# henriChevreux/distillation_trajectories

Hardware: AMD Instinct MI355X
Metric: trajectory-timesteps/sec (B×T U-Net fwd) at 16×16 T=50 (higher is better)
Workload: dtype f32 (fp32-accurate; convolutions: exact 3-plane bf16 operand split on bf16 MFMA with fp32 accumulate, or native fp32 MFMA, chosen per layer)

## Files before the change

### distillation_trajectories_amd/csrc/build.py

```python
import os
import shutil
import subprocess
import sys

HERE = os.path.dirname(os.path.abspath(__file__))
SOURCES = ["dt_conv.hip", "dt_conv_bf16.hip", "dt_conv_strip.hip", "dt_layers.hip", "dt_update.hip", "dt_metrics.hip", "dt_fused.hip", "dt_profile.hip", "dt_unet.hip",
           "dt_unet_forward.hip", "dt_unet_tune.hip", "dt_sample.hip", "dt_featnet.hip", "dt_inception.hip", "dt_pca.hip", "dt_fid.hip", "dt_lpips.hip", "dt_tsne.hip", "dt_quality.hip", "dt_quality_stream.hip", "dt_edit.hip", "dt_rng.hip"]
HEADERS = ["dt_internal.h", "dt_conv_forms.h", "dt_conv_rows.h", "dt_batch.h", "dt_dense64.h", "dt_quality_math.h", "dt_featnet.h", "dt_conv_epilogue.h", "dt_conv_walk.h", "dt_update_math.h", "dt_fused.h", "dt_unet.h", "dt_unet_layout.h", os.path.join("..", "..", "include", "dt_hip.h"),
           os.path.join("..", "..", "include", "dt_hip_noise.h"),
           os.path.join("..", "..", "include", "dt_hip_inception.h"),
           os.path.join("..", "..", "include", "dt_hip_pca.h"),
           os.path.join("..", "..", "include", "dt_hip_fid.h"),
           os.path.join("..", "..", "include", "dt_hip_fid_cov.h"),
           os.path.join("..", "..", "include", "dt_hip_lpips.h"),
           os.path.join("..", "..", "include", "dt_hip_tsne.h"),
           os.path.join("..", "..", "include", "dt_hip_quality.h"),
           os.path.join("..", "..", "include", "dt_hip_quality_stream.h"),
           os.path.join("..", "..", "include", "dt_hip_edit.h"),
           os.path.join("..", "..", "include", "dt_hip_rng.h")]
LIB = os.path.join(HERE, "libdt_hip.so")
ARCH = "gfx950"


def hipcc_path():
    for cand in (os.environ.get("HIPCC"), "/opt/rocm/bin/hipcc", shutil.which("hipcc")):
        if cand and os.path.exists(cand):
            return cand
    raise RuntimeError("hipcc not found (looked at $HIPCC, /opt/rocm/bin/hipcc, PATH)")


OBJ_DIR = os.path.join(HERE, "_build")
FLAGS = [f"--offload-arch={ARCH}", "-O3", "-std=c++17", "-fPIC", "-Wall", "-Wno-unused-function"]


def _newer(target, deps):
    if not os.path.exists(target):
        return True
    t = os.path.getmtime(target)
    return any(os.path.getmtime(d) > t for d in deps)


def is_stale():
    deps = [os.path.join(HERE, f) for f in SOURCES + HEADERS] + [os.path.abspath(__file__)]
    return _newer(LIB, deps)


def build(force=False, verbose=False):
    if not force and not is_stale():
        return LIB
    from concurrent.futures import ThreadPoolExecutor
    os.makedirs(OBJ_DIR, exist_ok=True)
    hipcc = hipcc_path()
    common = [os.path.join(HERE, f) for f in HEADERS] + [os.path.abspath(__file__)]

    def compile_one(src):
        obj = os.path.join(OBJ_DIR, src.replace(".hip", ".o"))
        path = os.path.join(HERE, src)
        if not force and not _newer(obj, [path] + common):
            return obj, None
# ... 85 lines not shown
```

### distillation_trajectories_amd/csrc/dt_conv.hip

```cpp
#include "dt_conv_walk.h"

namespace dt {

template <int BM, int BN>
__global__ __launch_bounds__(256, 4) void conv_gemm_kernel(const ConvParams p) {
  constexpr ConvForm F = *find_conv_form(KIND_FP32, BM, BN);
  constexpr int WN = F.wn();
  constexpr int MI = F.mi(), NI = F.ni();
  constexpr int A_PER = BM / 64, B_PER = BN / 64;
  constexpr int STAGE = (BM + BN) * 16;
  constexpr int LDS_FLOATS = 2 * STAGE > F.stage_floats() ? 2 * STAGE : F.stage_floats();
  static_assert(F.wm() == 2 && WN == 2 && MI * 64 == BM && NI * 64 == BN && LDS_FLOATS >= F.stage_floats(), "wave layout, epilogue stage");
  __shared__ __attribute__((aligned(16))) float lds[LDS_FLOATS];

  const int tid = threadIdx.x, lane = tid & 63, wave = tid >> 6;
  const int wm = wave / WN, wn = wave % WN;
  const int half = lane >> 5, l31 = lane & 31;
  const int m0 = blockIdx.x * BM, n0 = blockIdx.y * BN;
  const int HW = p.H * p.W;
  const ConvRowMath rm = kernarg_row_math();

  int a_off[A_PER], a_off2[A_PER], a_y[A_PER], a_x[A_PER];
  bool a_ok[A_PER];
  int a_lds[A_PER];
// ... 50 lines not shown
      for (int j = 0; j < B_PER; ++j) rb[j] = *reinterpret_cast<const f32x4 *>(wt + j * 1024);
      k.next();
    }
    if (it >= 0) {
      if (k.at_midpoint(p, it)) conv_midpoint<MI, NI>(p, acc, n0, wn, l31);
      const float *A = lds + (it & 1) * STAGE, *B = A + BM * 16;
#pragma unroll
      for (int s = 0; s < 2; ++s) {
        f32x4 fa[MI], fb[NI];
#pragma unroll
        for (int mi = 0; mi < MI; ++mi)
          fa[mi] = *reinterpret_cast<const f32x4 *>(A + a_row[mi] * 16 + (((2 * s + half) ^ ((a_row[mi] >> 2) & 3)) << 2));
#pragma unroll
        for (int ni = 0; ni < NI; ++ni)
          fb[ni] = *reinterpret_cast<const f32x4 *>(B + b_row[ni] * 16 + (((2 * s + half) ^ ((b_row[ni] >> 2) & 3)) << 2));
#pragma unroll
        for (int i = 0; i < 4; ++i)
#pragma unroll
          for (int mi = 0; mi < MI; ++mi)
#pragma unroll
            for (int ni = 0; ni < NI; ++ni) {
              acc[mi][ni] = __builtin_amdgcn_mfma_f32_32x32x2f32(fa[mi][i], fb[ni][i], acc[mi][ni], 0, 0, 0);
            }
      }
    }
    if (more) {
      float *A = lds + ((it + 1) & 1) * STAGE, *B = A + BM * 16;
#pragma unroll
      for (int j = 0; j < A_PER; ++j) *reinterpret_cast<f32x4 *>(A + a_lds[j]) = ra[j];
#pragma unroll
      for (int j = 0; j < B_PER; ++j) *reinterpret_cast<f32x4 *>(B + (tid + j * 256) * 4) = rb[j];
    }
    __syncthreads();
  }

  conv_epilogue<BM, BN, 1, false, true>(p, acc, lds, m0, n0, wm, wn, half, l31);
}

int launch_splitk_epilogue(const ConvParams &p, hipStream_t s);

#define DT_GEMM_ROW(cls, kind, bm, bn, kc, wk) {{kind, bm, bn, kc, wk, cls}, conv_gemm_kernel<bm, bn>},
static const ConvKernel kGemmKernels[] = {DT_CONV_FORMS_FP32(DT_GEMM_ROW)};

int launch_conv(const ConvParams &p_in, hipStream_t s) {
  ConvParams p = p_in;
  if (!p.in || !p.w || !p.scale || !p.shift || !p.out) return DT_E_NULL;
  if (p.H < 1 || p.W < 1) return DT_E_SHAPE;
  p.rm = make_row_math(p.H, p.W, p.m_per_tb, p.x3_imgs);
  if (p.cin_p % 16 || p.cout_p % 16 || p.n_p % kNPad || p.M <= 0) return DT_E_SHAPE;
  if ((long long)p.M * p.cin_p >= (1ll << 31) || (long long)p.M * p.cout_p * (p.n_dup > 1 ? p.n_dup : 1) >= (1ll << 31)) return DT_E_SHAPE;
  if (const int st = conv_admissible(p)) return st;
  {
    const double flops = 2.0 * p.M * (double)p.cout_real * ((double)p.cin_real * p.ksize * p.ksize + (p.in2 ? p.cin2_real : 0));
    ProfileScope prof(find_conv_form(p.kind, p.bm, p.bn)->cls, flops, 4.0 * p.M * ((double)p.cin_real + p.cout_real), s);
    if (p.kind == KIND_FP32) {
      conv_kernel_of(kGemmKernels, p).fn<<<dim3((p.M + p.bm - 1) / p.bm, p.n_p / p.bn, p.splits), 256, 0, s>>>(p);
      DT_LAUNCH_CHECK();
    } else if (const int st = is_strip(p.kind) ? launch_conv_strip(p, s) : launch_conv_bf16x6(p, s)) return st;
  }
  return p.splits > 1 ? launch_splitk_epilogue(p, s) : DT_OK;
}


bool conv_choice_valid(const ConvChoice &c, int slot, int n_p) {
  if (!find_conv_form(c.kind, c.bm, c.bn) || n_p % c.bn) return false;
  if (c.splits < 1 || c.splits > 9 || c.splits == 5 || c.splits == 6 || c.splits == 7) return false;
  return !c.fuse || (slot == 2 && c.splits == 1);
}

static ConvChoice heuristic_choice(int M, int n_p, int taps) {
  ConvChoice c{};
  c.bn = n_p % 128 == 0 ? 128 : 64;
  const long long blocks128 = (long long)((M + 127) / 128) * (n_p / c.bn);
  c.bm = blocks128 >= 512 ? 128 : 64;
  const long long blocks = (long long)((M + c.bm - 1) / c.bm) * (n_p / c.bn);
  c.splits = 1;
  if (taps == 9 && M <= kSplitMaxRows && blocks < 384) c.splits = blocks * 3 >= 384 ? 3 : 9;
  c.fuse = c.splits == 1;
  return c;
}

ConvChoice resolve_conv_choice(const ConvLayer &L, const ConvChoice *req, int precision) {
  ConvChoice c = req ? *req : heuristic_choice(L.M, L.n_p, L.splittable ? L.taps : 1);
  const int cc = L.cin_p >> 4;
  if (!req) {
    c.kind = precision == DT_PREC_FP32 ? KIND_FP32 : KIND_BF16;
    if (c.kind == KIND_BF16 && L.taps == 9 && strip_reaches(L.W)) {
      c.kind = KIND_STRIP;
      c.splits = c.splits == 9 ? (cc % 8 == 0 ? 8 : (cc % 4 == 0 ? 4 : 1)) : (c.splits == 3 ? (cc % 4 == 0 ? 4 : (cc % 2 == 0 ? 2 : 1)) : 1);
    }
  }
  if (c.kind == 2) c.kind = KIND_BF16;
  if (is_strip(c.kind) && (L.taps != 9 || !strip_reaches(L.W))) c.kind = KIND_BF16;
  if (c.kind == KIND_STRIPK && !find_conv_form(c.kind, c.bm, c.bn)) c.kind = KIND_STRIP2;
  if (c.bm == 256 && !find_conv_form(c.kind, c.bm, c.bn)) c.bm = 128;
  if (!L.splittable) c.splits = 1;
  const ConvForm *f = find_conv_form(c.kind, c.bm, c.bn);
  if (is_strip(c.kind) ? !chunks_fit(cc, pack_chunks(L.cin_p), c.splits * (f ? f->kc : 1)) : (L.taps * cc) % c.splits != 0)
    c.splits = 1;
  c.fuse = L.foldable && c.fuse && c.splits == 1;
  return c;
}

int conv_admissible(const ConvParams &p) {
  const int cc = p.cin_p >> 4;
  const ConvForm *f = find_conv_form(p.kind, p.bm, p.bn);
  if (!f || p.n_p % p.bn) return DT_E_ARG;
  if (p.splits < 1 || (p.splits > 1 && !p.slab)) return DT_E_ARG;
  if (p.ccw < cc || (p.in2 && p.ccw2 < (p.cin2_p >> 4))) return DT_E_ARG;
  if (p.in2 && (p.splits != 1 || !p.w2 || !p.bias2 || p.cin2_p % 16)) return DT_E_ARG;
  if (!is_strip(p.kind)) return (p.tap_hi - p.tap_lo) * cc % p.splits ? DT_E_ARG : DT_OK;
  if (p.ksize != 3 || p.tap_lo != 0 || p.tap_hi != 9 || !chunks_fit(cc, p.ccw, p.splits * f->kc)) return DT_E_ARG;
  if (p.in2 && !chunks_fit(p.cin2_p >> 4, p.ccw2, f->kc)) return DT_E_ARG;
  return f->reaches(p.W) ? DT_OK : DT_E_SHAPE;
}

template <int S>
__device__ inline float4 splitk_finish(const ConvParams &p, unsigned m, int n, size_t slab_stride) {
  const size_t o = (size_t)m * p.cout_p + n;
  float4 a;
  if (S > 0) {
    float4 part[S > 0 ? S : 1];
#pragma unroll
    for (int z = 0; z < S; ++z) part[z] = *reinterpret_cast<const float4 *>(p.slab + z * slab_stride + o);
    a = part[0];
#pragma unroll
    for (int z = 1; z < S; ++z) { a.x += part[z].x; a.y += part[z].y; a.z += part[z].z; a.w += part[z].w; }
  } else {
    a = *reinterpret_cast<const float4 *>(p.slab + o);
    for (int z = 1; z < p.splits; ++z) {
      const float4 b = *reinterpret_cast<const float4 *>(p.slab + z * slab_stride + o);
      a.x += b.x; a.y += b.y; a.z += b.z; a.w += b.w;
    }
  }
  const float4 sc = *reinterpret_cast<const float4 *>(p.scale + n), sh = *reinterpret_cast<const float4 *>(p.shift + n);
  float4 v = make_float4(a.x * sc.x + sh.x, a.y * sc.y + sh.y, a.z * sc.z + sh.z, a.w * sc.w + sh.w);
  if (p.relu) { v.x = fmaxf(v.x, 0.f); v.y = fmaxf(v.y, 0.f); v.z = fmaxf(v.z, 0.f); v.w = fmaxf(v.w, 0.f); }
  if (p.tb) {
    const float4 t = *reinterpret_cast<const float4 *>(p.tb + (size_t)row_tb((int)m, p.rm) * p.tb_stride + n);
    v.x += t.x; v.y += t.y; v.z += t.z; v.w += t.w;
  }
  if (p.add) {
    const float4 t = *reinterpret_cast<const float4 *>(p.add + o);
    v.x += t.x; v.y += t.y; v.z += t.z; v.w += t.w;
  }
  *reinterpret_cast<float4 *>(p.out + o) = v;
  return v;
}

template <int S, bool POOL>
__global__ __launch_bounds__(256) void splitk_epilogue_kernel(const ConvParams p) {
  const unsigned c4 = (unsigned)p.cout_p >> 2;
  const size_t slab_stride = (size_t)p.M * p.cout_p;
  const bool pow2 = (c4 & (c4 - 1)) == 0;
  const int sh4 = 31 - __builtin_clz(c4);
  if (!POOL) {
    const unsigned total = (unsigned)p.M * c4;
    for (unsigned i = blockIdx.x * blockDim.x + threadIdx.x; i < total; i += gridDim.x * blockDim.x) {
// ... 114 lines not shown
```

### distillation_trajectories_amd/csrc/dt_conv_forms.h

```cpp
#pragma once
#include <stddef.h>

namespace dt {

enum ConvKind {
  KIND_FP32 = 0,
  KIND_BF16 = 1,
  KIND_STRIP = 3,
  KIND_STRIP2 = 4,
  KIND_STRIPK = 5,
};
constexpr bool is_strip(int kind) { return kind >= KIND_STRIP; }

constexpr int strip_halo(int W, int bm) { return bm % W == 0 ? W : W + 1; }

constexpr int conv_real_channel(int cp, int cin, int cin_p, int split_c, int split_cp) {
  return cp < split_cp ? (cp < split_c ? cp : -1) : (cp < cin_p && split_c + (cp - split_cp) < cin ? split_c + (cp - split_cp) : -1);
}

enum ConvClass {
  KC_CONV_128x128 = 0, KC_CONV_128x64, KC_CONV_64x128, KC_CONV_64x64,
  KC_CONVB_128x128, KC_CONVB_128x64, KC_CONVB_64x128, KC_CONVB_64x64,
  KC_CONVS_128x128, KC_CONVS_128x64, KC_CONVS_64x128, KC_CONVS_64x64, KC_CONVS_256x64, KC_CONVS_K128x64, KC_CONVS_K64x64, KC_CONVS_K64x128,
  KC_CONV_COUNT
};

#define DT_CONV_FORMS_FP32(X)                    \
  X(KC_CONV_128x128, KIND_FP32, 128, 128, 1, 1)  \
  X(KC_CONV_128x64, KIND_FP32, 128, 64, 1, 1)    \
  X(KC_CONV_64x128, KIND_FP32, 64, 128, 1, 1)    \
  X(KC_CONV_64x64, KIND_FP32, 64, 64, 1, 1)
#define DT_CONV_FORMS_BF16(X)                    \
  X(KC_CONVB_128x128, KIND_BF16, 128, 128, 1, 1) \
  X(KC_CONVB_128x64, KIND_BF16, 128, 64, 1, 1)   \
  X(KC_CONVB_64x128, KIND_BF16, 64, 128, 1, 1)   \
  X(KC_CONVB_64x64, KIND_BF16, 64, 64, 1, 1)
#define DT_CONV_FORMS_STRIPK(X)                   \
  X(KC_CONVS_K64x128, KIND_STRIPK, 64, 128, 2, 2) \
  X(KC_CONVS_K64x64, KIND_STRIPK, 64, 64, 4, 4)   \
  X(KC_CONVS_K128x64, KIND_STRIPK, 128, 64, 2, 2)
#define DT_CONV_FORMS_STRIP2(X)                    \
  X(KC_CONVS_256x64, KIND_STRIP2, 256, 64, 2, 1)   \
  X(KC_CONVS_128x128, KIND_STRIP2, 128, 128, 2, 1) \
  X(KC_CONVS_128x64, KIND_STRIP2, 128, 64, 2, 1)   \
  X(KC_CONVS_64x128, KIND_STRIP2, 64, 128, 2, 1)   \
  X(KC_CONVS_64x64, KIND_STRIP2, 64, 64, 2, 1)
#define DT_CONV_FORMS_STRIP(X)                    \
  X(KC_CONVS_256x64, KIND_STRIP, 256, 64, 1, 1)   \
  X(KC_CONVS_128x128, KIND_STRIP, 128, 128, 1, 1) \
  X(KC_CONVS_128x64, KIND_STRIP, 128, 64, 1, 1)   \
  X(KC_CONVS_64x128, KIND_STRIP, 64, 128, 1, 1)   \
  X(KC_CONVS_64x64, KIND_STRIP, 64, 64, 1, 1)
#define DT_CONV_FORMS_ALL_STRIP(X) DT_CONV_FORMS_STRIPK(X) DT_CONV_FORMS_STRIP2(X) DT_CONV_FORMS_STRIP(X)

struct ConvForm {
  int kind, bm, bn, kc, wk, cls;

  constexpr int wn() const { return wk > 1 ? bn / 64 : (bm == 256 ? 1 : 2); }
  constexpr int wm() const { return 4 / (wn() * wk); }
  constexpr int mi() const { return bm / (32 * wm()); }
  constexpr int ni() const { return bn / (32 * wn()); }
  constexpr int kw() const { return kc / wk; }

  constexpr int ap() const { return bm == 256 ? 3 : (kc == 4 ? 1 : 2); }
  constexpr int max_w() const { return kc == 4 ? 31 : 63; }
// ... 44 lines not shown
```

### distillation_trajectories_amd/csrc/dt_internal.h

```cpp
#pragma once
#include <hip/hip_runtime.h>
#include <stddef.h>
#include <stdint.h>

#include "../../include/dt_hip.h"
#include "dt_conv_forms.h"
#include "dt_conv_rows.h"
#include "dt_unet_layout.h"

#define DT_HIP_TRY(expr)                         \
  do {                                           \
    hipError_t _e = (expr);                      \
    if (_e != hipSuccess) return (int)_e;        \
  } while (0)
#define DT_LAUNCH_CHECK()                        \
  do {                                           \
    hipError_t _e = hipGetLastError();           \
    if (_e != hipSuccess) return (int)_e;        \
  } while (0)

namespace dt {

enum KernelClass {
  KC_SPLITK_EPILOGUE = KC_CONV_COUNT, KC_FIRST_CONV, KC_POOL, KC_UPCAT, KC_HEAD, KC_HEAD_UP, KC_TIME_BIAS, KC_UPDATE, KC_METRICS,
  KC_WASSERSTEIN, KC_RESAMPLE, KC_FUSED, KC_PAIR_METRICS,
  KC_COUNT
};
struct ProfileScope {
  ProfileScope(int cls, double flops, double bytes, hipStream_t s);
  ~ProfileScope();
  int slot;
  hipStream_t stream;
  void *end_event;
};
bool profiling_on();

__device__ inline void bilinear_src(int dst, int in, int out, int &i0, int &i1, float &l0, float &l1) {
#pragma clang fp contract(off)
  const float scale = out > 1 ? (float)(in - 1) / (float)(out - 1) : 0.f;
  const float src = scale * (float)dst;
  i0 = (int)src;
  i1 = i0 + (i0 < in - 1 ? 1 : 0);
  l1 = src - (float)i0;
  l0 = 1.f - l1;
}
__device__ inline float bilinear_blend(float v00, float v01, float v10, float v11, float wy0, float wy1, float wx0, float wx1) {
  const float top = fmaf(wx1, v01, wx0 * v00), bot = fmaf(wx1, v11, wx0 * v10);
  return fmaf(wy1, bot, wy0 * top);
}

inline int grid_blocks(size_t total, int cap) { return (int)((total + 255) / 256 < (size_t)cap ? (total + 255) / 256 : (size_t)cap); }
inline bool chunks_fit(int cc, int ccw, int div) { return div >= 1 && round_up(cc, div) <= ccw; }

struct ConvParams {
  const float *in;
  const float *w;
  const float *scale;
  const float *shift;
  const float *tb;
  const float *add;
  float *out;
  int M, H, W;
  int cin_p, cout_p, n_p;
  int cin_real, cout_real;
  int ksize;
  int tap_lo, tap_hi;
  int relu;
  int tb_stride;
  int m_per_tb;
  int splits;
  float *slab;
  int bm, bn;
  int kind;
  const float *x3;
  const float *w3;
  int x3_hw, x3_imgs, x3_c;
  const float *in2;
  const float *w2;
  const float *bias2;
  int cin2_p, cin2_real;
  float *pool_out;
  const float *in_b, *in2_b;
  int cc_a, b_stride;
  const float *head_w, *head_b;
  float *head_out;
  int head_c, head_cin;
  const float *tbc;
  int n_dup, dup_rows;
  int dup_skip;
  int skip_out;
  int dup_stage2;
  int ccw, ccw2;
  ConvRowMath rm;
};

int launch_conv(const ConvParams &p, hipStream_t s);
int launch_conv_bf16x6(const ConvParams &p, hipStream_t s);
int launch_conv_strip(const ConvParams &p, hipStream_t s);
struct ConvKernel { ConvForm form; void (*fn)(ConvParams); };
template <size_t N>
inline const ConvKernel &conv_kernel_of(const ConvKernel (&table)[N], const ConvParams &p) {
  for (const ConvKernel &k : table)
    if (k.form.kind == p.kind && k.form.bm == p.bm && k.form.bn == p.bn) return k;
  return table[0];
}
int launch_pack_conv_bf16x3(const float *w_oihw, void *wp, int cout, int cin, int ksize, int cin_p, int cin_w, int n_p,
                            int split_c, int split_cp, hipStream_t s);

struct ConvChoice { int bm, bn, splits, kind, fuse; };
struct ConvLayer {
  int M, W;
  int n_p, cin_p;
  int taps;
  bool splittable;
  bool foldable;
};
inline bool strip_reaches(int W) { return find_conv_form(KIND_STRIP, 64, 64)->reaches(W); }
bool conv_choice_valid(const ConvChoice &c, int slot, int n_p);
ConvChoice resolve_conv_choice(const ConvLayer &L, const ConvChoice *req, int precision);
int conv_admissible(const ConvParams &p);

int launch_pack_conv(const float *w_oihw, float *wp, int cout, int cin, int ksize, int cin_p, int n_p,
                     int split_c, int split_cp, hipStream_t s);
int launch_fold_bn(const float *conv_b, const float *g, const float *b, const float *mean, const float *var,
                   float *scale, float *shift, int cout, int n_p, hipStream_t s);
int launch_pack_linear_rows(const float *w, const float *b, float *wp, float *bp, int out, int in, int out_p,
                            hipStream_t s);

int launch_first_conv(const float *x, const float *wf, const float *scale, const float *shift, const float *tb, int tb_stride,
                      int tb_div, float *out, int B, int n_pass, int C, int H, int W, int cout, int cout_p, hipStream_t s);
int launch_pack_first_conv(const float *w_oihw, float *wf, int cout, int C, int cout_p, hipStream_t s);
int launch_pack_tap_major(const float *w_oihw, float *w2t, int cout, int cin, int cp, hipStream_t s);
int launch_maxpool(const float *in, float *out, int Bt, int H, int W, int cp, hipStream_t s);
int launch_upcat(const float *lo, const float *skip, float *out, int Bt, int h, int w, int c1p, int c2p,
                 hipStream_t s);
int launch_head(const float *lo, const float *w, const float *bias, float *lowres, int Bt, int h, int w_, int cp, int C, int c_real,
                hipStream_t s);
int launch_head_upsample(const float *lowres, float *eps, int Bt, int h, int w_, int C, hipStream_t s);
int launch_pack_res3(const float *w, const float *b, float *w3, int cout, int C, int n_p, hipStream_t s);
struct MaskArgs {
  const float *mask;
  const int32_t *mask_row;
  const float *known;
  const int32_t *known_row;
};
int launch_cfg_update_lowres(int rule, const float *x, const float *lowres_u, const float *lowres_c, const float *z,
                             const int32_t *z_row, long long z_shift, const float coef[4], int has_noise, const float *w,
                             float w_scalar, float *out, int B, int C, int H, int W, int b_single, hipStream_t s,
                             const MaskArgs &mk = MaskArgs{});

struct TembWeights {
  const float *freqs;
  const float *w1, *b1;
  const float *wc0, *bc0;
  const float *wc2, *bc2;
  const float *wt, *bt;
  int D, half, tb_stride;
  int tb_cols;
  const float *w2t;
  int c0p;
};
int launch_time_bias(const TembWeights &tw, const int32_t *t, const float *cond, const uint8_t *present, int rows,
                     float *out, hipStream_t s);

}
```

### distillation_trajectories_amd/csrc/dt_profile.hip

```cpp
#include <atomic>
#include <mutex>
#include <vector>

#include "dt_internal.h"

using namespace dt;

namespace {
struct ProfRecord { hipEvent_t a, b; int cls; double flops, bytes; };
struct Profiler {
  std::mutex mu;
  std::atomic<bool> on{false};
  std::vector<ProfRecord> rec;
  std::vector<hipEvent_t> pool;
  size_t used = 0;
  hipEvent_t get() {
    if (used == pool.size()) {
      hipEvent_t e;
      if (hipEventCreate(&e) != hipSuccess) return nullptr;
      pool.push_back(e);
    }
    return pool[used++];
  }
} g_prof;
const char *kClassName[KC_COUNT - KC_CONV_COUNT] = {
    "splitk_epilogue_kernel", "first_conv_kernel", "maxpool_kernel", "upcat_kernel", "head_kernel", "head_upsample_kernel",
    "time_bias_kernel", "cfg_update_kernel", "traj_metrics_kernel", "wasserstein_kernel", "resampled_distance_kernel",
    "unet_fused_kernel", "pair_metrics_kernel"};
const char *class_name(int cls) {
  switch (cls) {
#define DT_GEMM(c, kind, bm, bn, kc, wk) case c: return "conv_gemm_kernel<" #bm "," #bn ">";
#define DT_BF16(c, kind, bm, bn, kc, wk) case c: return "conv_gemm_bf16x6_kernel<" #bm "," #bn ">";
#define DT_STRIP(c, kind, bm, bn, kc, wk) case c: return "conv_strip_bf16x6_kernel<" #bm "," #bn ">";
#define DT_STRIPK(c, kind, bm, bn, kc, wk) case c: return "conv_strip_bf16x6_kernel<" #bm "," #bn ",K" #kc ">";
    DT_CONV_FORMS_FP32(DT_GEMM) DT_CONV_FORMS_BF16(DT_BF16) DT_CONV_FORMS_STRIP(DT_STRIP) DT_CONV_FORMS_STRIPK(DT_STRIPK)
    default: return kClassName[cls - KC_CONV_COUNT];
  }
}
}

namespace dt {
ProfileScope::ProfileScope(int cls, double flops, double bytes, hipStream_t s) : slot(-1), stream(s), end_event(nullptr) {
  if (!g_prof.on.load(std::memory_order_relaxed)) return;
  hipEvent_t a;
  {
    std::lock_guard<std::mutex> lock(g_prof.mu);
    if (!g_prof.on.load(std::memory_order_relaxed)) return;
    a = g_prof.get();
    hipEvent_t b = g_prof.get();
    if (!a || !b) return;
    g_prof.rec.push_back(ProfRecord{a, b, cls, flops, bytes});
    slot = (int)g_prof.rec.size() - 1;
    end_event = b;
  }
  (void)hipEventRecord(a, s);
}
ProfileScope::~ProfileScope() {
  if (slot < 0) return;
  (void)hipEventRecord((hipEvent_t)end_event, stream);
}
bool profiling_on() { return g_prof.on.load(); }
}

extern "C" {

__global__ void profile_marker_kernel(int) {}

int dt_profile_marker(int id, void *stream) {
  profile_marker_kernel<<<1, 64, 0, (hipStream_t)stream>>>(id);
  DT_LAUNCH_CHECK();
  return DT_OK;
}

int dt_profile_begin(void) {
  std::lock_guard<std::mutex> lock(g_prof.mu);
  g_prof.rec.clear();
  g_prof.used = 0;
  g_prof.on = true;
  return DT_OK;
}

// ... 25 lines not shown
```

### distillation_trajectories_amd/csrc/dt_unet.h

```cpp
#pragma once
#include <mutex>
#include <vector>

#include "dt_fused.h"

namespace dt {

struct ConvW {
  float *w, *wb;
  float *scale, *shift;
};
struct BlockW {
  ConvW c[3];
  float *w3;
};

struct TunedShape {
  FwdShape shape;
  ConvChoice c[kBlocks][3];
};

struct LoopGraph {
  std::vector<unsigned char> key;
  hipGraphExec_t exec = nullptr;
  hipGraph_t graph = nullptr;
  LoopGraph() = default;
  LoopGraph(LoopGraph &&o) noexcept : key(std::move(o.key)), exec(o.exec), graph(o.graph) { o.exec = nullptr; o.graph = nullptr; }
  LoopGraph &operator=(LoopGraph &&o) noexcept {
    std::swap(key, o.key); std::swap(exec, o.exec); std::swap(graph, o.graph);
    return *this;
  }
  ~LoopGraph() {
    if (exec) (void)hipGraphExecDestroy(exec);
    if (graph) (void)hipGraphDestroy(graph);
  }
};

class GraphCache {
 public:
  static constexpr size_t kMax = 8;
  std::mutex mu;
  const LoopGraph *find(const std::vector<unsigned char> &key) const {
    for (const LoopGraph &g : graphs)
      if (g.key == key) return &g;
    return nullptr;
  }
  const LoopGraph &insert(LoopGraph &&g) {
    if (graphs.size() >= kMax) graphs.erase(graphs.begin());
    graphs.push_back(std::move(g));
    return graphs.back();
  }
  size_t size() const { return graphs.size(); }
  void clear() {
    std::lock_guard<std::mutex> lock(mu);
    graphs.clear();
  }
 private:
  std::vector<LoopGraph> graphs;
};

}

struct dt_unet {
  dt_unet() = default;
  dt_unet(const dt_unet &) = delete;
  dt_unet &operator=(const dt_unet &) = delete;
  ~dt_unet() {
    graphs.clear();
    if (slab) (void)hipFree(slab);
    if (fused_slab) (void)hipFree(fused_slab);
  }
  std::vector<dt::TunedShape> tuned;
  mutable dt::GraphCache graphs;
  int precision = DT_PREC_AUTO;
  bool head_fusion = true;
  dt::UnetGeom geo{};
  dt::BlockW blk[dt::kBlocks] = {};
  float *slab = nullptr;
  dt::TembWeights tw{};
  const float *final_w = nullptr, *final_b = nullptr;
  bool fused_ok = false, fused_on = false;
  int fused_G = 2;
  float *fused_slab = nullptr;
  dt::FusedOp *fused_ops_dev = nullptr;
  int fused_n_ops = 0;
  dt::FusedLds fused_lds{};
  int fused_par = 0, fused_n_par = 0;
};

namespace dt {

const TunedShape *find_tuned(const dt_unet *u, const FwdShape &sh);
TunedShape *tuned_for(dt_unet *u, const FwdShape &sh);

struct ResolvedForward {
  FwdShape shape;
  bool shared_enc1;
  ConvChoice c[kBlocks][3];
  bool pool_fused[kBlocks];
  bool concat_in_place[kBlocks];
  bool head_fused;
};
ConvLayer conv_layer(const dt_unet *u, const ResolvedForward &f, int j, int slot);
ResolvedForward resolve_forward(const dt_unet *u, const FwdShape &sh, const TunedShape *tuned);
ConvParams bind_conv(const dt_unet *u, const ResolvedForward &f, int j, int slot, const ConvChoice &c, const float *in, float *ws,
                     const Plan &pl, const float *tb, int tb_div);
int forward_impl(const dt_unet *u, const float *x, const BatchSplit &b, int H, int W, const float *tb, float *eps, float *ws,
                 size_t ws_bytes, hipStream_t s);
bool use_fused(const dt_unet *u, int H, int W);
void fused_common(const dt_unet *u, FusedArgs &a, const BatchSplit &b, const float *tb);

}
```

### distillation_trajectories_amd/csrc/dt_unet.hip

```cpp
#include <cstdlib>
#include <memory>
#include <new>

#include "dt_unet.h"

using namespace dt;

namespace {

constexpr int kSlotWeight[3] = {DT_BT_RES_W, DT_BT_CONV1_W, DT_BT_CONV2_W};

struct SlabWriter {
  float *base;
  hipStream_t s;
  int st = DT_OK;
  float *at(size_t off) const { return base + off; }
  void copy(size_t off, const float *src, size_t n) {
    if (st != DT_OK) return;
    const hipError_t e = hipMemcpyAsync(base + off, src, n * sizeof(float), hipMemcpyDeviceToDevice, s);
    if (e != hipSuccess) st = (int)e;
  }
};

int pack_slab(dt_unet *u, const SlabLayout &L, const float *const *bt, const float *const *gt, hipStream_t s) {
// ... 87 lines not shown
      *fc[slot] = FusedConvW{(int)o_w[j][slot], scale, shift};
      if (st == DT_OK && g.has_launch(j, slot))
        st = launch_pack_fused_conv(t[kSlotWeight[slot]], wr.at(o_w[j][slot]), k.cout, cg.cin, cg.ksize * cg.ksize, cg.cin_p / 16, k.cout_p / 16,
                                    cg.split_c, cg.split_cp, s);
    }
    pj += 5 * cp;
  }
  if (st == DT_OK && hipMemsetAsync(wr.at(o_par + 4 * c0p), 0, sizeof(float) * c0p, s) != hipSuccess) st = (int)hipGetLastError();
  u->fused_par = (int)o_par; u->fused_n_par = n_par;
  if (st != DT_OK) return st;
  FusedOp ops[kFusedMaxOps];
  u->fused_n_ops = fused_ops(m, G, ops);
  u->fused_ops_dev = reinterpret_cast<FusedOp *>(wr.at(o_ops));
  DT_HIP_TRY(hipMemcpy(u->fused_ops_dev, ops, sizeof(FusedOp) * u->fused_n_ops, hipMemcpyHostToDevice));
  u->fused_lds = lds;
  u->fused_ok = true;
  u->fused_on = getenv("DT_NO_FUSED") == nullptr;
  return DT_OK;
}

}

extern "C" {

int dt_abi_version(void) { return DT_ABI_VERSION; }

const char *dt_status_string(int st) {
  switch (st) {
    case DT_OK: return "ok";
    case DT_E_NULL: return "required pointer is NULL";
    case DT_E_SHAPE: return "unsupported or inconsistent shape";
    case DT_E_ARG: return "bad enum or count";
    case DT_E_WORKSPACE: return "workspace too small";
    default: return st > 0 ? hipGetErrorString((hipError_t)st) : "unknown dt status";
  }
}

int dt_unet_create(const dt_unet_desc *desc, const float *const *bt, const float *const *gt, void *stream,
                   dt_unet **out) {
  if (!desc || !bt || !gt || !out) return DT_E_NULL;
  UnetGeom geo;
  if (const int bad = unet_geometry(*desc, getenv("DT_NO_SHARED_ENC1") == nullptr, &geo)) return bad;
  for (int i = 0; i < DT_GT_COUNT; ++i)
    if (!gt[i]) return DT_E_NULL;
  for (int j = 0; j < kBlocks; ++j)
    for (int t = 0; t < DT_BT_COUNT; ++t) {
      const bool optional = t == DT_BT_RES_W || t == DT_BT_RES_B;
      if (!bt[j * DT_BT_COUNT + t] && (!optional || geo.blk[j].has_res)) return DT_E_NULL;
    }
  hipStream_t s = (hipStream_t)stream;
  std::unique_ptr<dt_unet> u(new (std::nothrow) dt_unet());
  if (!u) return (int)hipErrorOutOfMemory;
  u->geo = geo;
  const SlabLayout L = slab_layout(geo);
  DT_HIP_TRY(hipMalloc((void **)&u->slab, L.total * sizeof(float)));
  if (const int st = pack_slab(u.get(), L, bt, gt, s)) return st;
  if (const int st = build_fused(u.get(), bt, s)) return st;
  *out = u.release();
  return DT_OK;
}

void dt_unet_destroy(dt_unet *h) { delete h; }

int dt_unet_time_bias_stride(const dt_unet *h) { return h ? h->geo.tb_stride : DT_E_NULL; }

int dt_unet_time_bias(const dt_unet *h, const int32_t *t, const float *cond, const uint8_t *present, int rows,
                      float *out, void *stream) {
  if (!h || !t || !out) return DT_E_NULL;
  if (rows < 0) return DT_E_ARG;
  return launch_time_bias(h->tw, t, cond, present, rows, out, (hipStream_t)stream);
}

size_t dt_unet_workspace_bytes(const dt_unet *h, int batch_total, int H, int W) {
  const FwdShape sh = FwdShape::rows_only(batch_total, H, W);
  if (!h || sh.validate() != DT_OK) return 0;
  return make_plan(h->geo, sh).total * sizeof(float);
}

int dt_unet_debug_activation(const dt_unet *h, int batch_total, int H, int W, int which, size_t *off, int *cp,
                             int *oh, int *ow) {
  if (!h || !off || !cp || !oh || !ow) return DT_E_NULL;
  if (which < 0 || which > kBlocks) return DT_E_ARG;
  const FwdShape sh = FwdShape::rows_only(batch_total, H, W);
  if (const int bad = sh.validate()) return bad;
  const Plan pl = make_plan(h->geo, sh);
  if (which == kBlocks) { *off = pl.slab; *cp = 0; *oh = 0; *ow = 0; return DT_OK; }
  *off = pl.o[which]; *cp = h->geo.blk[which].cout_p; *oh = pl.H[which]; *ow = pl.W[which];
  return DT_OK;
}

int dt_unet_set_precision(dt_unet *h, int precision) {
  if (!h) return DT_E_NULL;
  if (precision < DT_PREC_FP32 || precision > DT_PREC_AUTO) return DT_E_ARG;
  h->tuned.clear();
  h->graphs.clear();
  h->precision = precision;
  return DT_OK;
}

int dt_unet_set_head_fusion(dt_unet *h, int on) {
  if (!h) return DT_E_NULL;
  h->head_fusion = on != 0;
  h->graphs.clear();
  return DT_OK;
}

// ... 14 lines not shown
```

### distillation_trajectories_amd/csrc/dt_unet_forward.hip

```cpp
#include "dt_unet.h"

namespace dt {

const TunedShape *find_tuned(const dt_unet *u, const FwdShape &sh) {
  for (const TunedShape &t : u->tuned)
    if (t.shape == sh) return &t;
  return nullptr;
}

TunedShape *tuned_for(dt_unet *u, const FwdShape &sh) {
  for (TunedShape &t : u->tuned)
    if (t.shape == sh) return &t;
  return nullptr;
}

ConvLayer conv_layer(const dt_unet *u, const ResolvedForward &f, int j, int slot) {
  const BlockGeom &k = u->geo.blk[j];
  const int h = f.shape.H / kDiv[j], w = f.shape.W / kDiv[j];
  const int M = (j == 0 && f.shared_enc1 ? f.shape.imgs : f.shape.Bt) * h * w;
  const int taps = slot == 0 || (h == 1 && w == 1) ? 1 : 9;
  return ConvLayer{M, w, k.n_p, k.c[slot].cin_p, taps, j > 0 && M <= kSplitMaxRows, slot == 2 && j > 0 && k.has_res};
}

ResolvedForward resolve_forward(const dt_unet *u, const FwdShape &sh, const TunedShape *tuned) {
  const UnetGeom &g = u->geo;
  ResolvedForward f{};
  f.shape = sh;
  f.shared_enc1 = g.share_enc1 && (sh.Bt + sh.single) % sh.imgs == 0;
  for (int j = 0; j < kBlocks; ++j)
    for (int slot = 0; slot < 3; ++slot)
      if (g.has_launch(j, slot)) f.c[j][slot] = resolve_conv_choice(conv_layer(u, f, j, slot), tuned ? &tuned->c[j][slot] : nullptr, u->precision);
  for (int j = 0; j < kBlocks; ++j) {
    const ConvChoice &c2 = f.c[j][2];
    const int h = sh.H / kDiv[j], w = sh.W / kDiv[j];
    f.pool_fused[j] = j <= 3 && h % 2 == 0 && w % 2 == 0 && (c2.splits > 1 || (w <= 16 && (w & (w - 1)) == 0));
    f.concat_in_place[j] = j >= 5 && g.blk[j].has_res && is_strip(f.c[j][1].kind) && is_strip(c2.kind) && c2.fuse;
  }
  const ConvChoice &last = f.c[kBlocks - 1][2];
  f.head_fused = u->head_fusion && last.splits == 1 && g.blk[kBlocks - 1].n_p == last.bn && g.desc.channels <= 3;
  return f;
}

ConvParams bind_conv(const dt_unet *u, const ResolvedForward &f, int j, int slot, const ConvChoice &c, const float *in, float *ws,
                     const Plan &pl, const float *tb, int tb_div) {
  const UnetGeom &g = u->geo;
  const BlockGeom &k = g.blk[j];
  const ConvGeom &cg = k.c[slot];
  const ConvW &cw = u->blk[j].c[slot];
  const ConvLayer L = conv_layer(u, f, j, slot);
  const int h = pl.H[j], w = pl.W[j];
  ConvParams p{};
  p.M = L.M; p.H = h; p.W = w;
  p.cin_p = L.cin_p; p.cout_p = k.cout_p; p.n_p = k.n_p;
  p.cin_real = cg.cin; p.cout_real = k.cout;
  p.tb_stride = g.tb_stride; p.m_per_tb = h * w * tb_div;
  p.slab = ws + pl.slab;
  p.in = slot == 2 ? ws + pl.h[j] : in;
  p.ksize = cg.ksize;
  p.scale = cw.scale; p.shift = cw.shift;
  p.tap_lo = slot > 0 && L.taps == 1 ? 4 : 0; p.tap_hi = p.tap_lo + L.taps;
  p.relu = slot > 0;
  if (slot == 0) {
    p.out = ws + pl.r[j];
  } else if (slot == 1) {
    p.tb = tb + k.tb_off; p.out = ws + pl.h[j];
  } else {
    p.out = ws + pl.o[j];
    if (f.pool_fused[j]) p.pool_out = ws + pl.pool[j];
    if (j == 0) {
      p.x3 = in; p.w3 = u->blk[0].w3; p.x3_hw = h * w; p.x3_imgs = f.shape.imgs; p.x3_c = g.desc.channels;
      if (f.shared_enc1) {
        p.n_dup = (f.shape.Bt + f.shape.single) / f.shape.imgs; p.dup_rows = p.M; p.dup_skip = f.shape.single * h * w; p.tbc = tb + g.tb_cols;
        p.skip_out = u->head_fusion && p.pool_out ? 1 : 0;
      }
// ... 127 lines not shown
```

### distillation_trajectories_amd/csrc/dt_unet_tune.hip

```cpp
#include <algorithm>
#include <cstring>

#include "dt_unet.h"

using namespace dt;

namespace {

struct ConvTimer {
  hipEvent_t e0 = nullptr, e1 = nullptr;
  ~ConvTimer() {
    if (e0) (void)hipEventDestroy(e0);
    if (e1) (void)hipEventDestroy(e1);
  }
  int create() {
    DT_HIP_TRY(hipEventCreate(&e0));
    DT_HIP_TRY(hipEventCreate(&e1));
    return DT_OK;
  }
  int time(const ConvParams &q, int reps, hipStream_t s, float *ms) {
    *ms = 0.f;
    int st = launch_conv(q, s);
    if (st != DT_OK) return st;
    (void)hipEventRecord(e0, s);
// ... 26 lines not shown
            if (sp > 1 && tiles * (sp / 2) >= 1024) continue;
            out.push_back(ConvChoice{bm, bn, sp, kind, fuse});
          }
      }
  }
  return out;
}

}

extern "C" {

int dt_unet_autotune(dt_unet *h, int batch_total, int H, int W, int images, int single, void *workspace, size_t ws_bytes,
                     void *stream) {
  if (!h || !workspace) return DT_E_NULL;
  TunedShape t{{batch_total, H, W, images, single}, {}};
  if (const int bad = t.shape.validate()) return bad;
  hipStream_t s = (hipStream_t)stream;
  const Plan pl = make_plan(h->geo, t.shape);
  if (pl.total * sizeof(float) > ws_bytes) return DT_E_WORKSPACE;
  float *ws = (float *)workspace;
  ConvTimer timer;
  if (const int bad = timer.create()) return bad;
  const ResolvedForward f = resolve_forward(h, t.shape, nullptr);
  const float *tb = h->slab;
  int st = DT_OK;
  {
    const ConvParams wp = bind_conv(h, f, 1, 1, f.c[1][1], ws + pl.input(1), ws, pl, tb, batch_total);
    for (int rep = 0; rep < 200 && st == DT_OK; ++rep) st = launch_conv(wp, s);
    if (hipStreamSynchronize(s) != hipSuccess) st = (int)hipGetLastError();
  }
  auto measure = [&](const ConvParams &q, int reps) -> float {
    float ms;
    const int lst = timer.time(q, reps, s, &ms);
    if (lst != DT_OK && lst != DT_E_SHAPE && lst != DT_E_ARG) st = lst;
    return lst == DT_OK ? ms : -1.f;
  };
  for (int j = 0; j < kBlocks && st == DT_OK; ++j) {
    const float *in = ws + pl.input(j);
    float skip_ms = 0.f;
    for (int slot = 0; slot < 3 && st == DT_OK; ++slot) {
      if (!h->geo.has_launch(j, slot)) continue;
      ConvChoice best = f.c[j][slot];
      best.fuse = 0;
      const ConvLayer L = conv_layer(h, f, j, slot);
      float best_ms = 1e30f;
      struct Cand { ConvChoice c; ConvParams q; float cost; };
      std::vector<Cand> cands;
      auto cost_of = [&](float ms, const ConvChoice &c) {
        return (ms + (c.fuse ? 0.f : (L.foldable ? skip_ms : 0.f))) * (c.splits > 1 ? kSplitMargin : 1.0f);
      };
      const bool feeds_head = j == kBlocks - 1 && slot == 2 && h->head_fusion && h->geo.desc.channels <= 3;
      for (const ConvChoice &c : tune_candidates(L, h->precision, feeds_head)) {
        const ConvParams q = bind_conv(h, f, j, slot, c, in, ws, pl, tb, batch_total);
        if (conv_admissible(q) != DT_OK) continue;
        const float ms = measure(q, 3);
        if (ms < 0.f) continue;
        cands.push_back(Cand{c, q, cost_of(ms, c)});
      }
      if (!cands.empty() && st == DT_OK) {
        std::vector<size_t> top;
        for (size_t i = 0; i < cands.size(); ++i) top.push_back(i);
        std::stable_sort(top.begin(), top.end(), [&](size_t a, size_t b) { return cands[a].cost < cands[b].cost; });
        if (top.size() > 3) top.resize(3);
        std::sort(top.begin(), top.end());
        std::vector<float> fin(top.size(), 1e30f);
        for (int round = 0; round < 2 && st == DT_OK; ++round)
          for (size_t k = 0; k < top.size() && st == DT_OK; ++k) {
            const float ms = measure(cands[top[k]].q, 10);
            if (ms >= 0.f && ms < fin[k]) fin[k] = ms;
          }
        for (size_t k = 0; k < top.size(); ++k) {
          const float cost = cost_of(fin[k], cands[top[k]].c);
          if (cost < best_ms * 1.01f) { best_ms = cost < best_ms ? cost : best_ms; best = cands[top[k]].c; }
        }
      }
      t.c[j][slot] = best;
      if (slot == 0) skip_ms = best_ms;
    }
  }
  if (st != DT_OK) return st;
  if (TunedShape *old = tuned_for(h, t.shape)) *old = t;
  else h->tuned.push_back(t);
  h->graphs.clear();
  return DT_OK;
}

int dt_unet_time_conv(const dt_unet *h, int batch_total, int H, int W, int images, int single, int block, int slot, int bm,
                      int bn, int splits, int prec, int fuse, int reps, void *workspace, size_t ws_bytes, void *stream,
                      float *ms, double *flops) {
  if (!h || !workspace || !ms || !flops) return DT_E_NULL;
  if (!slot_exists(block, slot) || reps < 1) return DT_E_ARG;
  TunedShape req{{batch_total, H, W, images, single}, {}};
  if (const int bad = req.shape.validate()) return bad;
  const Plan pl = make_plan(h->geo, req.shape);
  if (pl.total * sizeof(float) > ws_bytes) return DT_E_WORKSPACE;
  float *ws = (float *)workspace;
  if (!h->geo.has_launch(block, slot)) { *ms = 0.f; *flops = 0.0; return DT_OK; }
  std::fill_n(&req.c[0][0], kBlocks * 3, ConvChoice{bm, bn, splits, prec, fuse});
  const ResolvedForward f = resolve_forward(h, req.shape, &req);
  const ConvParams p = bind_conv(h, f, block, slot, f.c[block][slot], ws + pl.input(block), ws, pl, h->slab, batch_total);
  *flops = 2.0 * p.M * (double)p.cout_real * ((double)p.cin_real * p.ksize * p.ksize + (p.in2 ? p.cin2_real : 0));
  ConvTimer timer;
  if (const int bad = timer.create()) return bad;
  return timer.time(p, reps, (hipStream_t)stream, ms);
}

int dt_unet_conv_choice(const dt_unet *h, int batch_total, int H, int W, int images, int single, int block, int slot, int *bm,
                        int *bn, int *splits, int *prec, int *tuned) {
  if (!h || !bm || !bn || !splits || !prec || !tuned) return DT_E_NULL;
  if (!slot_exists(block, slot)) return DT_E_ARG;
  const FwdShape sh{batch_total, H, W, images, single};
  if (const int bad = sh.validate()) return bad;
  const TunedShape *t = find_tuned(h, sh);
  const ResolvedForward f = resolve_forward(h, sh, t);
  const ConvChoice &c = f.c[block][slot];
  *bm = c.bm; *bn = c.bn; *splits = c.splits; *prec = c.kind + (c.fuse ? 8 : 0); *tuned = t && h->geo.has_launch(block, slot);
  if (slot == 0 && f.c[block][2].fuse) *bm = *bn = *splits = 0;
  return DT_OK;
}

int dt_unet_set_conv_choice(dt_unet *h, int batch_total, int H, int W, int images, int single, int block, int slot, int bm,
                            int bn, int splits, int prec, int fuse) {
  if (!h) return DT_E_NULL;
  if (!slot_exists(block, slot)) return DT_E_ARG;
  const FwdShape sh{batch_total, H, W, images, single};
  if (const int bad = sh.validate()) return bad;
  const ConvChoice c{bm, bn, splits, prec, fuse};
  if (!conv_choice_valid(c, slot, h->geo.blk[block].n_p)) return DT_E_ARG;
  TunedShape *t = tuned_for(h, sh);
  if (!t) {
    TunedShape fresh{sh, {}};
    memcpy(fresh.c, resolve_forward(h, sh, nullptr).c, sizeof(fresh.c));
    h->tuned.push_back(fresh);
    t = &h->tuned.back();
  }
  t->c[block][slot] = c;
  h->graphs.clear();
  return DT_OK;
}

}
```

Before: 359,700.

## Add register-pipelined low-resolution GEMM kernel for small 1x1 and center-tap convs

Adds a dedicated LDS-free GEMM kernel for small-M layers: 1-tap or center-tap convolutions at low resolution with bf16 split-precision MFMA. Each wave computes a 32x32 tile and prefetches 8 K-groups of activations and weight planes into registers ahead of use. When the layer is lowres, uses the bf16 kind, has one tap, few rows and no fusion, the launcher selects this kernel instead of the generic tiled one, aiming to cut LDS staging and tile-padding overhead on tiny GEMMs. The kernel is on by default and can be disabled with an environment variable. It sums split-K slices inside the kernel and does its epilogue directly.

```diff
diff --git a/distillation_trajectories_amd/csrc/build.py b/distillation_trajectories_amd/csrc/build.py
--- a/distillation_trajectories_amd/csrc/build.py
+++ b/distillation_trajectories_amd/csrc/build.py
@@ -4,7 +4,7 @@
 import sys
 
 HERE = os.path.dirname(os.path.abspath(__file__))
-SOURCES = ["dt_conv.hip", "dt_conv_bf16.hip", "dt_conv_strip.hip", "dt_layers.hip", "dt_update.hip", "dt_metrics.hip", "dt_fused.hip", "dt_profile.hip", "dt_unet.hip",
+SOURCES = ["dt_conv.hip", "dt_conv_bf16.hip", "dt_conv_strip.hip", "dt_lowres.hip", "dt_layers.hip", "dt_update.hip", "dt_metrics.hip", "dt_fused.hip", "dt_profile.hip", "dt_unet.hip",
            "dt_unet_forward.hip", "dt_unet_tune.hip", "dt_sample.hip", "dt_featnet.hip", "dt_inception.hip", "dt_pca.hip", "dt_fid.hip", "dt_lpips.hip", "dt_tsne.hip", "dt_quality.hip", "dt_quality_stream.hip", "dt_edit.hip", "dt_rng.hip"]
 HEADERS = ["dt_internal.h", "dt_conv_forms.h", "dt_conv_rows.h", "dt_batch.h", "dt_dense64.h", "dt_quality_math.h", "dt_featnet.h", "dt_conv_epilogue.h", "dt_conv_walk.h", "dt_update_math.h", "dt_fused.h", "dt_unet.h", "dt_unet_layout.h", os.path.join("..", "..", "include", "dt_hip.h"),
            os.path.join("..", "..", "include", "dt_hip_noise.h"),
diff --git a/distillation_trajectories_amd/csrc/dt_conv.hip b/distillation_trajectories_amd/csrc/dt_conv.hip
--- a/distillation_trajectories_amd/csrc/dt_conv.hip
+++ b/distillation_trajectories_amd/csrc/dt_conv.hip
@@ -126,7 +126,9 @@
   if (const int st = conv_admissible(p)) return st;
   {
     const double flops = 2.0 * p.M * (double)p.cout_real * ((double)p.cin_real * p.ksize * p.ksize + (p.in2 ? p.cin2_real : 0));
-    ProfileScope prof(find_conv_form(p.kind, p.bm, p.bn)->cls, flops, 4.0 * p.M * ((double)p.cin_real + p.cout_real), s);
+    ProfileScope prof(p.kind == KIND_LOWRES ? (int)KC_LOWRES_GEMM : find_conv_form(p.kind, p.bm, p.bn)->cls, flops,
+                      4.0 * p.M * ((double)p.cin_real + p.cout_real), s);
+    if (p.kind == KIND_LOWRES) return launch_lowres_gemm(p, s);
     if (p.kind == KIND_FP32) {
       conv_kernel_of(kGemmKernels, p).fn<<<dim3((p.M + p.bm - 1) / p.bm, p.n_p / p.bn, p.splits), 256, 0, s>>>(p);
       DT_LAUNCH_CHECK();
@@ -164,7 +166,7 @@
       c.splits = c.splits == 9 ? (cc % 8 == 0 ? 8 : (cc % 4 == 0 ? 4 : 1)) : (c.splits == 3 ? (cc % 4 == 0 ? 4 : (cc % 2 == 0 ? 2 : 1)) : 1);
     }
   }
-  if (c.kind == 2) c.kind = KIND_BF16;
+  if (c.kind == 2 || c.kind == KIND_LOWRES) c.kind = KIND_BF16;
   if (is_strip(c.kind) && (L.taps != 9 || !strip_reaches(L.W))) c.kind = KIND_BF16;
   if (c.kind == KIND_STRIPK && !find_conv_form(c.kind, c.bm, c.bn)) c.kind = KIND_STRIP2;
   if (c.bm == 256 && !find_conv_form(c.kind, c.bm, c.bn)) c.bm = 128;
@@ -173,11 +175,21 @@
   if (is_strip(c.kind) ? !chunks_fit(cc, pack_chunks(L.cin_p), c.splits * (f ? f->kc : 1)) : (L.taps * cc) % c.splits != 0)
     c.splits = 1;
   c.fuse = L.foldable && c.fuse && c.splits == 1;
+  return conv_launch_kind(L, c);
+}
+
+ConvChoice conv_launch_kind(const ConvLayer &L, ConvChoice c) {
+  if (L.lowres && c.kind == KIND_BF16 && L.taps == 1 && L.M <= kSplitMaxRows && !c.fuse) c.kind = KIND_LOWRES;
   return c;
 }
 
 int conv_admissible(const ConvParams &p) {
   const int cc = p.cin_p >> 4;
+  if (p.kind == KIND_LOWRES) {
+    if (p.tap_hi - p.tap_lo != 1 || (p.ksize == 3 ? p.tap_lo != 4 || p.H != 1 || p.W != 1 : p.ksize != 1 || p.tap_lo != 0)) return DT_E_ARG;
+    if (p.in2 || p.in_b || p.x3 || p.n_dup || p.pool_out || p.head_out || p.ccw < cc) return DT_E_ARG;
+    return p.splits >= 1 && cc % p.splits == 0 ? DT_OK : DT_E_ARG;
+  }
   const ConvForm *f = find_conv_form(p.kind, p.bm, p.bn);
   if (!f || p.n_p % p.bn) return DT_E_ARG;
   if (p.splits < 1 || (p.splits > 1 && !p.slab)) return DT_E_ARG;
diff --git a/distillation_trajectories_amd/csrc/dt_conv_forms.h b/distillation_trajectories_amd/csrc/dt_conv_forms.h
--- a/distillation_trajectories_amd/csrc/dt_conv_forms.h
+++ b/distillation_trajectories_amd/csrc/dt_conv_forms.h
@@ -9,8 +9,9 @@
   KIND_STRIP = 3,
   KIND_STRIP2 = 4,
   KIND_STRIPK = 5,
+  KIND_LOWRES = 6,
 };
-constexpr bool is_strip(int kind) { return kind >= KIND_STRIP; }
+constexpr bool is_strip(int kind) { return kind >= KIND_STRIP && kind <= KIND_STRIPK; }
 
 constexpr int strip_halo(int W, int bm) { return bm % W == 0 ? W : W + 1; }
 
diff --git a/distillation_trajectories_amd/csrc/dt_internal.h b/distillation_trajectories_amd/csrc/dt_internal.h
--- a/distillation_trajectories_amd/csrc/dt_internal.h
+++ b/distillation_trajectories_amd/csrc/dt_internal.h
@@ -23,7 +23,7 @@
 
 enum KernelClass {
   KC_SPLITK_EPILOGUE = KC_CONV_COUNT, KC_FIRST_CONV, KC_POOL, KC_UPCAT, KC_HEAD, KC_HEAD_UP, KC_TIME_BIAS, KC_UPDATE, KC_METRICS,
-  KC_WASSERSTEIN, KC_RESAMPLE, KC_FUSED, KC_PAIR_METRICS,
+  KC_WASSERSTEIN, KC_RESAMPLE, KC_FUSED, KC_PAIR_METRICS, KC_LOWRES_GEMM,
   KC_COUNT
 };
 struct ProfileScope {
@@ -97,6 +97,7 @@
 int launch_conv(const ConvParams &p, hipStream_t s);
 int launch_conv_bf16x6(const ConvParams &p, hipStream_t s);
 int launch_conv_strip(const ConvParams &p, hipStream_t s);
+int launch_lowres_gemm(const ConvParams &p, hipStream_t s);
 struct ConvKernel { ConvForm form; void (*fn)(ConvParams); };
 template <size_t N>
 inline const ConvKernel &conv_kernel_of(const ConvKernel (&table)[N], const ConvParams &p) {
@@ -114,10 +115,12 @@
   int taps;
   bool splittable;
   bool foldable;
+  bool lowres;
 };
 inline bool strip_reaches(int W) { return find_conv_form(KIND_STRIP, 64, 64)->reaches(W); }
 bool conv_choice_valid(const ConvChoice &c, int slot, int n_p);
 ConvChoice resolve_conv_choice(const ConvLayer &L, const ConvChoice *req, int precision);
+ConvChoice conv_launch_kind(const ConvLayer &L, ConvChoice c);
 int conv_admissible(const ConvParams &p);
 
 int launch_pack_conv(const float *w_oihw, float *wp, int cout, int cin, int ksize, int cin_p, int n_p,
diff --git a/distillation_trajectories_amd/csrc/dt_lowres.hip b/distillation_trajectories_amd/csrc/dt_lowres.hip
--- /dev/null
+++ b/distillation_trajectories_amd/csrc/dt_lowres.hip
@@ -0,0 +1,116 @@
+#include "dt_conv_epilogue.h"
+
+namespace dt {
+
+constexpr int kLowresAhead = 8;
+
+__global__ __launch_bounds__(256) void lowres_gemm_kernel(const ConvParams p) {
+  const int lane = threadIdx.x & 63, wave = threadIdx.x >> 6;
+  const int half = lane >> 5, l31 = lane & 31;
+  const int tn = blockIdx.y * 4 + wave;
+  if (tn >= (p.n_p >> 5)) return;
+  const int m0 = blockIdx.x * 32, n0 = tn * 32;
+  const int n = n0 + l31;
+
+  const int m_a = m0 + l31 < p.M ? m0 + l31 : 0;
+  const float *a_lane = p.in + (size_t)m_a * p.cin_p + half * 8;
+  const size_t w_plane = (size_t)p.n_p * 16;
+  const __bf16 *w_lane = reinterpret_cast<const __bf16 *>(p.w) + (size_t)p.tap_lo * p.ccw * 3 * w_plane + (size_t)n * 16 +
+                         ((half ^ ((n >> 3) & 1)) << 3);
+
+  const int n_total = p.cin_p >> 4;
+  const int n_main = n_total / p.splits;
+  const int n_ring = n_total - n_total % kLowresAhead;
+
+  const int n_sc = n < p.cout_p ? n : 0;
+  const float sc = p.scale[n_sc], sh = p.shift[n_sc];
+  f32x16 acc, sum;
+#pragma unroll
+  for (int r = 0; r < 16; ++r) { acc[r] = 0.f; sum[r] = 0.f; }
+  int in_slice = 0;
+  bool first_slice = true;
+
+  f32x4 ra[kLowresAhead][2];
+  bf16x8 rb[kLowresAhead][3];
+  auto request = [&](f32x4 (&a)[2], bf16x8 (&b)[3], int g) __attribute__((always_inline)) {
+    const float *src = a_lane + g * 16;
+    a[0] = *reinterpret_cast<const f32x4 *>(src);
+    a[1] = *reinterpret_cast<const f32x4 *>(src + 4);
+    const __bf16 *wt = w_lane + (size_t)g * 3 * w_plane;
+#pragma unroll
+    for (int pl = 0; pl < 3; ++pl) b[pl] = *reinterpret_cast<const bf16x8 *>(wt + pl * w_plane);
+  };
+  bf16x8 fa[2][3];
+  auto split = [&](const f32x4 (&a)[2], bf16x8 (&f)[3]) __attribute__((always_inline)) { split8(a[0], a[1], f[0], f[1], f[2]); };
+  auto multiply = [&](const bf16x8 (&f)[3], const bf16x8 (&b)[3]) __attribute__((always_inline)) {
+    mfma_bf16x6(acc, f, b);
+    if (++in_slice == n_main) {
+#pragma unroll
+      for (int r = 0; r < 16; ++r) {
+        sum[r] = first_slice ? acc[r] : sum[r] + acc[r];
+        acc[r] = 0.f;
+      }
+      first_slice = false;
+      in_slice = 0;
+    }
+  };
+
+  if (n_ring) {
+#pragma unroll
+    for (int d = 0; d < kLowresAhead; ++d) request(ra[d], rb[d], d);
+    split(ra[0], fa[0]);
+  }
+  for (int g0 = kLowresAhead; g0 < n_ring; g0 += kLowresAhead) {
+#pragma unroll
+    for (int d = 0; d < kLowresAhead; ++d) {
+      if (d + 1 < kLowresAhead) split(ra[d + 1], fa[(d + 1) & 1]);
+      multiply(fa[d & 1], rb[d]);
+      request(ra[d], rb[d], g0 + d);
+      if (d + 1 == kLowresAhead) split(ra[0], fa[0]);
+    }
+  }
+  if (n_ring) {
+#pragma unroll
+    for (int d = 0; d < kLowresAhead; ++d) {
+      if (d + 1 < kLowresAhead) split(ra[d + 1], fa[(d + 1) & 1]);
+      multiply(fa[d & 1], rb[d]);
+    }
+  }
+  for (int g = n_ring; g < n_total; ++g) {
+    f32x4 ta[2];
+    bf16x8 tb[3];
+    request(ta, tb, g);
+    split(ta, fa[0]);
+    multiply(fa[0], tb);
+  }
+
+  if (n >= p.cout_p) return;
+  float t[16], a[16];
+  unsigned o[16];
+  bool ok[16];
+#pragma unroll
+  for (int r = 0; r < 16; ++r) {
+    const int m = m0 + 4 * half + (r & 3) + 8 * (r >> 2);
+    ok[r] = m < p.M;
+    const int mm = ok[r] ? m : 0;
+    o[r] = (unsigned)mm * p.cout_p + n;
+    t[r] = p.tb ? p.tb[(size_t)row_tb(mm, p.rm) * p.tb_stride + n] : 0.f;
+    a[r] = p.add ? p.add[o[r]] : 0.f;
+  }
+#pragma unroll
+  for (int r = 0; r < 16; ++r) {
+    float v = sum[r] * sc + sh;
+    if (p.relu) v = fmaxf(v, 0.f);
+    if (p.tb) v += t[r];
+    if (p.add) v += a[r];
+    if (ok[r]) p.out[o[r]] = v;
+  }
+}
+
+int launch_lowres_gemm(const ConvParams &p, hipStream_t s) {
+  lowres_gemm_kernel<<<dim3((p.M + 31) / 32, ((p.n_p >> 5) + 3) / 4), 256, 0, s>>>(p);
+  DT_LAUNCH_CHECK();
+  return DT_OK;
+}
+
+}
diff --git a/distillation_trajectories_amd/csrc/dt_profile.hip b/distillation_trajectories_amd/csrc/dt_profile.hip
--- a/distillation_trajectories_amd/csrc/dt_profile.hip
+++ b/distillation_trajectories_amd/csrc/dt_profile.hip
@@ -26,7 +26,7 @@
 const char *kClassName[KC_COUNT - KC_CONV_COUNT] = {
     "splitk_epilogue_kernel", "first_conv_kernel", "maxpool_kernel", "upcat_kernel", "head_kernel", "head_upsample_kernel",
     "time_bias_kernel", "cfg_update_kernel", "traj_metrics_kernel", "wasserstein_kernel", "resampled_distance_kernel",
-    "unet_fused_kernel", "pair_metrics_kernel"};
+    "unet_fused_kernel", "pair_metrics_kernel", "lowres_gemm_kernel"};
 const char *class_name(int cls) {
   switch (cls) {
 #define DT_GEMM(c, kind, bm, bn, kc, wk) case c: return "conv_gemm_kernel<" #bm "," #bn ">";
diff --git a/distillation_trajectories_amd/csrc/dt_unet.h b/distillation_trajectories_amd/csrc/dt_unet.h
--- a/distillation_trajectories_amd/csrc/dt_unet.h
+++ b/distillation_trajectories_amd/csrc/dt_unet.h
@@ -74,6 +74,7 @@
   mutable dt::GraphCache graphs;
   int precision = DT_PREC_AUTO;
   bool head_fusion = true;
+  bool lowres_gemm = true;
   dt::UnetGeom geo{};
   dt::BlockW blk[dt::kBlocks] = {};
   float *slab = nullptr;
diff --git a/distillation_trajectories_amd/csrc/dt_unet.hip b/distillation_trajectories_amd/csrc/dt_unet.hip
--- a/distillation_trajectories_amd/csrc/dt_unet.hip
+++ b/distillation_trajectories_amd/csrc/dt_unet.hip
@@ -163,6 +163,7 @@
   std::unique_ptr<dt_unet> u(new (std::nothrow) dt_unet());
   if (!u) return (int)hipErrorOutOfMemory;
   u->geo = geo;
+  u->lowres_gemm = getenv("DT_NO_LOWRES_GEMM") == nullptr;
   const SlabLayout L = slab_layout(geo);
   DT_HIP_TRY(hipMalloc((void **)&u->slab, L.total * sizeof(float)));
   if (const int st = pack_slab(u.get(), L, bt, gt, s)) return st;
diff --git a/distillation_trajectories_amd/csrc/dt_unet_forward.hip b/distillation_trajectories_amd/csrc/dt_unet_forward.hip
--- a/distillation_trajectories_amd/csrc/dt_unet_forward.hip
+++ b/distillation_trajectories_amd/csrc/dt_unet_forward.hip
@@ -19,7 +19,7 @@
   const int h = f.shape.H / kDiv[j], w = f.shape.W / kDiv[j];
   const int M = (j == 0 && f.shared_enc1 ? f.shape.imgs : f.shape.Bt) * h * w;
   const int taps = slot == 0 || (h == 1 && w == 1) ? 1 : 9;
-  return ConvLayer{M, w, k.n_p, k.c[slot].cin_p, taps, j > 0 && M <= kSplitMaxRows, slot == 2 && j > 0 && k.has_res};
+  return ConvLayer{M, w, k.n_p, k.c[slot].cin_p, taps, j > 0 && M <= kSplitMaxRows, slot == 2 && j > 0 && k.has_res, u->lowres_gemm};
 }
 
 ResolvedForward resolve_forward(const dt_unet *u, const FwdShape &sh, const TunedShape *tuned) {
diff --git a/distillation_trajectories_amd/csrc/dt_unet_tune.hip b/distillation_trajectories_amd/csrc/dt_unet_tune.hip
--- a/distillation_trajectories_amd/csrc/dt_unet_tune.hip
+++ b/distillation_trajectories_amd/csrc/dt_unet_tune.hip
@@ -102,7 +102,7 @@
       };
       const bool feeds_head = j == kBlocks - 1 && slot == 2 && h->head_fusion && h->geo.desc.channels <= 3;
       for (const ConvChoice &c : tune_candidates(L, h->precision, feeds_head)) {
-        const ConvParams q = bind_conv(h, f, j, slot, c, in, ws, pl, tb, batch_total);
+        const ConvParams q = bind_conv(h, f, j, slot, conv_launch_kind(L, c), in, ws, pl, tb, batch_total);
         if (conv_admissible(q) != DT_OK) continue;
         const float ms = measure(q, 3);
         if (ms < 0.f) continue;
@@ -165,7 +165,8 @@
   const TunedShape *t = find_tuned(h, sh);
   const ResolvedForward f = resolve_forward(h, sh, t);
   const ConvChoice &c = f.c[block][slot];
-  *bm = c.bm; *bn = c.bn; *splits = c.splits; *prec = c.kind + (c.fuse ? 8 : 0); *tuned = t && h->geo.has_launch(block, slot);
+  *bm = c.bm; *bn = c.bn; *splits = c.splits; *tuned = t && h->geo.has_launch(block, slot);
+  *prec = (c.kind == KIND_LOWRES ? (int)KIND_BF16 : c.kind) + (c.fuse ? 8 : 0);
   if (slot == 0 && f.c[block][2].fuse) *bm = *bn = *splits = 0;
   return DT_OK;
 }
```

New measurement: 361,600 (median of 5 runs). Within noise of the previous version (+0.5%).
